# metagentools/VStrains

Measured on AMD Instinct MI355X. Metric: PE read pairs/sec through PE-link inference (GFA index + packed reads in HBM -> node_mat/short_mat), higher is better.
Workload: dtype u32

## Files before the change

include/vstrains_hip.h:

```cpp
#ifndef VSTRAINS_HIP_H
#define VSTRAINS_HIP_H

#include <stddef.h>
#include <stdint.h>

#ifdef __cplusplus
extern "C" {
#endif

#define VS_ABI_VERSION 10

enum {
    VS_OK = 0,
    VS_E_ARG = -1,
    VS_E_HIP = -2,
    VS_E_OOM = -3,
    VS_E_NODE_BASE = -4,
    VS_E_STATE = -5,
    VS_E_RANGE = -6,
    VS_E_UTF8 = -7,
    VS_E_KEY = -8,
    VS_E_FPE = -9,
    VS_E_RECURSION = -10
};
// ... 71 lines not shown
                   const uint32_t *cum, uint32_t n_strains, uint64_t seed, uint64_t first_pair,
                   uint64_t n_pairs, uint32_t read_len, uint32_t sub_thresh, uint32_t n_thresh,
                   vs_reads **out);

int vs_pe_count(vs_ctx *ctx, const vs_reads *reads, uint32_t *d_node_mat, uint32_t *d_short_mat,
                uint64_t *d_stats);

int vs_pe_count_tracked(vs_ctx *ctx, const vs_reads *reads, uint32_t *d_node_mat, uint32_t *d_short_mat,
                        uint64_t *d_stats, uint8_t *d_tile_map);
int vs_counts_zero_tracked(vs_ctx *ctx, uint32_t *d_node_mat, uint32_t *d_short_mat, uint32_t n, uint8_t *d_tile_map);

int vs_counts_fold(vs_ctx *ctx, uint32_t *d_counts, int64_t *d_wide, uint64_t n);

int vs_counts_occupied(vs_ctx *ctx, const void *d_cells, uint32_t cell_bytes, uint64_t n_stretches, uint8_t *d_occ);

int vs_comm_unique_id(vs_ctx *ctx, uint8_t id[128]);
int vs_comm_init_rank(vs_ctx *ctx, int n_ranks, const uint8_t id[128], int rank, void **comm);
int vs_comm_destroy(vs_ctx *ctx, void *comm);
int vs_pe_allreduce(vs_ctx *ctx, void *comm, void *d_node_mat, void *d_short_mat, uint64_t *d_stats,
                    uint32_t n, int wide);

int vs_pe_map_ends(vs_ctx *ctx, const vs_reads *reads, uint32_t cap, uint32_t *lists,
                   uint32_t *counts);

int vs_pe_last_timing(vs_ctx *ctx, double ms[5]);
const char *vs_pe_last_kernel(const vs_ctx *ctx);
enum {
    VS_RAN_LOCUS_LDS_SORT = 1,
    VS_RAN_LOCUS_GLOBAL_SORT = 2,
    VS_RAN_PE_MID = 8,
    VS_RAN_ROW_OWNERS = 16
};
uint32_t vs_pe_last_launched(const vs_ctx *ctx);

typedef struct vs_links vs_links;
int vs_links_from_counts(vs_ctx *ctx, const uint32_t *d_node_mat, const uint32_t *d_short_mat,
                         uint32_t n, vs_links **out);
int vs_links_from_counts_tracked(vs_ctx *ctx, const uint32_t *d_node_mat, const uint32_t *d_short_mat, uint32_t n,
                                 const uint8_t *d_tile_map, uint32_t sparse_min_nodes, vs_links **out);
int vs_links_from_wide(vs_ctx *ctx, const int64_t *d_node_mat, const int64_t *d_short_mat,
                       uint32_t n, vs_links **out);
int vs_links_from_host(vs_ctx *ctx, const int64_t *node_mat, const int64_t *short_mat, uint32_t n,
                       vs_links **out);
int vs_links_reserve(vs_ctx *ctx, uint32_t n);
void vs_links_free(vs_ctx *ctx, vs_links *links);
int vs_links_size(const vs_links *links, uint32_t *n);
int vs_links_to_host(vs_ctx *ctx, const vs_links *links, int64_t *out );
int vs_links_block_sums(vs_ctx *ctx, const vs_links *links, const uint64_t *list_off,
                        const uint32_t *list_idx, uint32_t n_lists, const uint32_t *qa,
                        const uint32_t *qb, uint64_t n_queries, int64_t *out);
int vs_links_group_matrix(vs_ctx *ctx, const vs_links *links, const uint64_t *list_off,
                          const uint32_t *list_idx, uint32_t n_groups, int64_t *out);

int vs_graph_refresh(vs_ctx *ctx, uint32_t n_vertices, uint32_t n_edge_slots,
                     const uint64_t *row_ptr, const uint32_t *n_out, const uint32_t *nbr,
                     const uint32_t *eidx, const double *dp, const uint8_t *vertex_black,
                     const uint8_t *edge_black, double *flow, uint8_t *nontrivial,
                     uint8_t *fork_kind, int32_t *chain_next, int32_t *chain_top,
                     int32_t *chain_rank, uint32_t *zero_sum_edge);

typedef struct vs_stage vs_stage;
enum {
    VS_STAGE_GRAPH = 1,
    VS_STAGE_CONTIGS = 2,
    VS_STAGE_LINKS = 4,
    VS_STAGE_STRAINS = 8,
// ... 38 lines not shown
```

vstrains_amd/_native.py:

```python
from __future__ import annotations

import ctypes as C
import os

_HERE = os.path.dirname(os.path.abspath(__file__))
LIB_PATH = os.path.join(_HERE, "libvstrains_hip.so")

VS_OK = 0
VS_E_ARG, VS_E_HIP, VS_E_OOM, VS_E_NODE_BASE, VS_E_STATE, VS_E_RANGE, VS_E_UTF8, VS_E_KEY, VS_E_FPE = -1, -2, -3, -4, -5, -6, -7, -8, -9

SYMBOLS = {
    "vs_abi_version": (C.c_int, []),
    "vs_device_count": (C.c_int, []),
    "vs_ctx_create": (C.c_int, [C.c_int, C.POINTER(C.c_void_p)]),
    "vs_ctx_destroy": (None, [C.c_void_p]),
    "vs_last_error": (C.c_char_p, [C.c_void_p]),
    "vs_ctx_set_stream": (C.c_int, [C.c_void_p, C.c_void_p]),
    "vs_ctx_sync": (C.c_int, [C.c_void_p]),
    "vs_index_build": (C.c_int, [C.c_void_p, C.c_void_p, C.c_void_p, C.c_uint32, C.c_uint32,
                                 C.POINTER(C.c_uint32), C.POINTER(C.c_uint8)]),
    "vs_index_info": (C.c_int, [C.c_void_p, C.POINTER(C.c_uint64)]),
    "vs_index_export": (C.c_int, [C.c_void_p, C.c_void_p, C.c_void_p, C.c_void_p, C.c_void_p, C.c_void_p, C.POINTER(C.c_uint64)]),
    "vs_node_order_host": (C.c_int, [C.c_void_p, C.c_void_p, C.c_uint32, C.c_uint32, C.c_void_p]),
    "vs_reads_pack": (C.c_int, [C.c_void_p, C.c_void_p, C.c_void_p, C.c_uint64, C.POINTER(C.c_void_p)]),
# ... 13 lines not shown
    "vs_fastq_block": (C.c_int, [C.c_void_p, C.c_void_p, C.c_uint64, C.c_uint64, C.POINTER(C.c_void_p)]),
    "vs_fastq_stream_open": (C.c_int, [C.c_void_p, C.c_char_p, C.c_char_p, C.POINTER(C.c_void_p)]),
    "vs_fastq_stream_next": (C.c_int, [C.c_void_p, C.c_void_p, C.c_uint64, C.POINTER(C.c_void_p), C.POINTER(C.c_uint64)]),
    "vs_fastq_stream_info": (C.c_int, [C.c_void_p, C.POINTER(C.c_uint64)]),
    "vs_fastq_stream_close": (None, [C.c_void_p]),
    "vs_fastq_scan_text": (C.c_int, [C.c_void_p, C.c_void_p, C.c_uint64, C.c_uint32, C.c_void_p, C.c_uint64, C.POINTER(C.c_uint64)]),
    "vs_bgzf_walk": (C.c_int, [C.c_void_p, C.c_uint64, C.c_void_p, C.c_uint64, C.POINTER(C.c_uint64)]),
    "vs_inflate_host": (C.c_int, [C.c_void_p, C.c_uint32, C.c_void_p, C.c_uint32, C.c_uint32, C.POINTER(C.c_uint32)]),
    "vs_inflate_bgzf": (C.c_int, [C.c_void_p, C.c_void_p, C.c_uint64, C.c_void_p, C.c_uint64, C.c_uint32, C.c_void_p, C.c_uint64,
                                  C.POINTER(C.c_uint64)]),
    "vs_fastq_stream_inflate_info": (C.c_int, [C.c_void_p, C.POINTER(C.c_uint64)]),
    "vs_bgzf_walk_file": (C.c_int, [C.c_char_p, C.c_void_p, C.c_uint64, C.POINTER(C.c_uint64)]),
    "vs_bgzf_count_lines": (C.c_int, [C.c_void_p, C.c_char_p, C.c_void_p, C.c_uint64, C.c_void_p, C.POINTER(C.c_uint64)]),
    "vs_inflate_count_host": (C.c_int, [C.c_void_p, C.c_uint32, C.c_uint32, C.c_uint32, C.POINTER(C.c_uint32)]),
    "vs_bgzf_shard_plan": (C.c_int, [C.c_void_p, C.c_uint64, C.c_int, C.c_uint64, C.c_uint64, C.POINTER(C.c_uint64)]),
    "vs_fastq_stream_open_range": (C.c_int, [C.c_void_p, C.c_char_p, C.c_char_p, C.POINTER(C.c_uint64), C.c_uint64, C.POINTER(C.c_void_p)]),
    "vs_write_matrix_text": (C.c_int, [C.c_void_p, C.c_char_p, C.c_void_p, C.c_void_p, C.c_uint32, C.c_void_p]),
    "vs_synth_pairs": (C.c_int, [C.c_void_p, C.c_void_p, C.c_void_p, C.c_void_p, C.c_uint32, C.c_uint64,
                                 C.c_uint64, C.c_uint64, C.c_uint32, C.c_uint32, C.c_uint32,
                                 C.POINTER(C.c_void_p)]),
    "vs_pe_count": (C.c_int, [C.c_void_p, C.c_void_p, C.c_void_p, C.c_void_p, C.c_void_p]),
    "vs_pe_count_tracked": (C.c_int, [C.c_void_p, C.c_void_p, C.c_void_p, C.c_void_p, C.c_void_p, C.c_void_p]),
    "vs_counts_zero_tracked": (C.c_int, [C.c_void_p, C.c_void_p, C.c_void_p, C.c_uint32, C.c_void_p]),
    "vs_counts_fold": (C.c_int, [C.c_void_p, C.c_void_p, C.c_void_p, C.c_uint64]),
    "vs_counts_occupied": (C.c_int, [C.c_void_p, C.c_void_p, C.c_uint32, C.c_uint64, C.c_void_p]),
    "vs_comm_unique_id": (C.c_int, [C.c_void_p, C.c_void_p]),
    "vs_comm_init_rank": (C.c_int, [C.c_void_p, C.c_int, C.c_void_p, C.c_int, C.POINTER(C.c_void_p)]),
    "vs_comm_destroy": (C.c_int, [C.c_void_p, C.c_void_p]),
    "vs_pe_allreduce": (C.c_int, [C.c_void_p, C.c_void_p, C.c_void_p, C.c_void_p, C.c_void_p, C.c_uint32, C.c_int]),
    "vs_pe_map_ends": (C.c_int, [C.c_void_p, C.c_void_p, C.c_uint32, C.c_void_p, C.c_void_p]),
    "vs_pe_last_kernel": (C.c_char_p, [C.c_void_p]),
    "vs_pe_last_launched": (C.c_uint32, [C.c_void_p]),
    "vs_pe_last_timing": (C.c_int, [C.c_void_p, C.POINTER(C.c_double)]),
    "vs_links_from_counts": (C.c_int, [C.c_void_p, C.c_void_p, C.c_void_p, C.c_uint32, C.POINTER(C.c_void_p)]),
    "vs_links_from_counts_tracked": (C.c_int, [C.c_void_p, C.c_void_p, C.c_void_p, C.c_uint32, C.c_void_p, C.c_uint32, C.POINTER(C.c_void_p)]),
    "vs_links_from_wide": (C.c_int, [C.c_void_p, C.c_void_p, C.c_void_p, C.c_uint32, C.POINTER(C.c_void_p)]),
    "vs_links_from_host": (C.c_int, [C.c_void_p, C.c_void_p, C.c_void_p, C.c_uint32, C.POINTER(C.c_void_p)]),
    "vs_links_reserve": (C.c_int, [C.c_void_p, C.c_uint32]),
    "vs_links_free": (None, [C.c_void_p, C.c_void_p]),
    "vs_links_size": (C.c_int, [C.c_void_p, C.POINTER(C.c_uint32)]),
    "vs_links_to_host": (C.c_int, [C.c_void_p, C.c_void_p, C.c_void_p]),
    "vs_links_block_sums": (C.c_int, [C.c_void_p, C.c_void_p, C.c_void_p, C.c_void_p, C.c_uint32, C.c_void_p,
                                      C.c_void_p, C.c_uint64, C.c_void_p]),
    "vs_links_group_matrix": (C.c_int, [C.c_void_p, C.c_void_p, C.c_void_p, C.c_void_p, C.c_uint32, C.c_void_p]),
    "vs_graph_refresh": (C.c_int, [C.c_void_p, C.c_uint32, C.c_uint32] + [C.c_void_p] * 13 + [C.POINTER(C.c_uint32)]),
    "vs_stage_create": (C.c_int, [C.c_void_p, C.c_void_p, C.POINTER(C.c_void_p)]),
    "vs_dev_alloc": (C.c_int, [C.c_void_p, C.c_size_t, C.POINTER(C.c_void_p)]),
    "vs_dev_free": (C.c_int, [C.c_void_p, C.c_void_p]),
    "vs_dev_zero": (C.c_int, [C.c_void_p, C.c_void_p, C.c_size_t]),
    "vs_dev_to_host": (C.c_int, [C.c_void_p, C.c_void_p, C.c_void_p, C.c_size_t]),
}

_lib = None


class NativeError(RuntimeError):
    def __init__(self, code: int, msg: str):
        super().__init__("libvstrains_hip: %s (code %d)" % (msg, code))
        self.code = code


def lib():
    global _lib
    if _lib is None:
        if not os.path.exists(LIB_PATH):
            raise ImportError(
# ... 20 lines not shown
```

vstrains_amd/csrc/vs_internal.h:

```cpp
#pragma once

#include <hip/hip_runtime.h>
#include <stdint.h>
#include <string>
#include <vector>

#include "../../include/vstrains_hip.h"
#include "vs_buf.h"
#include "vs_pe_plan.h"

#define VS_WAVE 64
#define VS_PAD_WORDS 16


struct VsNodeMeta {
    uint32_t woff;
    uint32_t len;
};

struct VsSlot {
    uint64_t key;
    uint32_t a;
    uint32_t b;
};
// ... 58 lines not shown

void vs_tuning_load(VsTuning &t, bool experiment);

struct vs_ctx {
    int device = 0;
    bool experiment = false;
    VsTuning tune;
    hipStream_t stream = nullptr;
    std::string err;
    FqStage fq_stage[2];
    unsigned fq_next = 0;
    bool has_index = false;
    VsIndexDev idx{};
    VsDevBuf d_meta, d_fwd, d_table, d_post;
    uint64_t n_seed_pos = 0, n_slots = 0, n_distinct = 0, index_bytes = 0;
    uint32_t max_node_len = 0;
    VsDevBuf d_slow_list;
    VsDevBuf d_slow_count;
    enum SlowCount : uint32_t {
        SC_MID = 0,
        SC_ACC_QUEUE = 1,
        SC_SLOW = 8,
        SC_STRIP_QUEUE = 9,
        SC_OWNERS = 15,
        SC_WORDS = 16
    };
    VsDevBuf links_spare;
    uint32_t links_spare_n = 0;
    VsDevBuf d_slow_list2;
    VsDevBuf d_dense;
    uint32_t dense_nodes = 0xFFFFFFFFu;
    VsDevBuf d_locus_keys, d_perm, d_locus_hist, d_scan_tmp;
    double last_sort_ms = 0;
    VsDevBuf d_lists, d_list_counts;
    VsDevBuf d_rows, d_row_entries, d_mult, d_ltab;
    VsDevBuf scratch[32];
    struct CachedBuf { VsDevBuf buf; bool used; };
    std::vector<CachedBuf> cache;
    hipEvent_t ev[5] = {nullptr, nullptr, nullptr, nullptr, nullptr};
    double last_ms[3] = {0, 0, 0};
    const char *last_kernel = "";
    uint32_t last_launched = 0;
    int n_cu = 256;
};

struct vs_reads {
    uint64_t n_ends = 0, n_words = 0, max_len = 0, n_invalid = 0, bytes = 0;
    void *d_woff = nullptr, *d_meta = nullptr, *d_words = nullptr, *d_mask = nullptr, *d_inv4 = nullptr;
    bool cached = false;
    VsDevBuf own[5];
    unsigned n_own = 0;
    hipError_t own_alloc(void *&view, size_t bytes) {
        const hipError_t e = own[n_own].reserve(bytes);
        view = own[n_own].ptr();
        if (e == hipSuccess) n_own++;
        return e;
    }
    VsReadsDev dev() const {
        VsReadsDev r;
        r.n_ends = n_ends;
        r.woff = (const uint32_t *)d_woff;
        r.meta = (const uint32_t *)d_meta;
        r.words = (const uint32_t *)d_words;
        r.mask = (const uint32_t *)d_mask;
        r.inv4 = (const uint32_t *)d_inv4;
        return r;
// ... 57 lines not shown
__device__ __forceinline__ uint64_t vs_win(const uint32_t *w, uint32_t base) { return vs_win64_u32(w, base); }
__device__ __forceinline__ uint64_t vs_win(const uint32_t *w, uint64_t base) { return vs_win64(w, base); }

__device__ __forceinline__ uint32_t vs_fastdiv(uint32_t x, uint32_t magic) { return magic ? __umulhi(x, magic) : x; }

__device__ __forceinline__ uint64_t vs_lowmask(uint32_t bits) {
    return bits >= 64u ? ~0ull : ((1ull << bits) - 1ull);
}

__device__ __forceinline__ uint64_t vs_rc(uint64_t x, uint32_t w) {
    x = __builtin_bitreverse64(x);
    x = ((x >> 1) & 0x5555555555555555ull) | ((x & 0x5555555555555555ull) << 1);
    return (~x) >> (64u - 2u * w);
}

__device__ __forceinline__ uint64_t vs_mix64(uint64_t z);
template <typename B>
__device__ __forceinline__ uint64_t vs_seed_key(const uint32_t *words, B base, uint32_t w, uint32_t *strand) {
    if (w <= 31u) {
        const uint64_t f = vs_win(words, base) & vs_lowmask(2u * w);
        const uint64_t r = vs_rc(f, w);
        *strand = r < f ? 1u : 0u;
        return r < f ? r : f;
    }
    const uint32_t sh = 2u * (w - 32u);
    const uint64_t lo = vs_win(words, base), hi = vs_win(words, base + (B)32) & vs_lowmask(sh);
    const uint64_t rl = vs_rc(lo, 32u), rh = vs_rc(hi, w - 32u);
    const uint64_t rc_lo = (rl << sh) | rh, rc_hi = sh ? rl >> (64u - sh) : 0ull;
    const bool rev = rc_hi < hi || (rc_hi == hi && rc_lo < lo);
    *strand = rev ? 1u : 0u;
    const uint64_t a = rev ? rc_lo : lo, b = rev ? rc_hi : hi;
    return vs_mix64(a ^ vs_mix64(b + 0x632BE59BD9B4E019ull)) >> 2;
}
template <typename B>
__device__ __forceinline__ bool vs_seed_dirty(const uint32_t *mask, B base, uint32_t w) {
    if (w <= 32u) return (vs_win(mask, base) & vs_lowmask(2u * w)) != 0ull;
    return vs_win(mask, base) != 0ull || (vs_win(mask, base + (B)32) & vs_lowmask(2u * (w - 32u))) != 0ull;
}

__device__ __forceinline__ uint32_t vs_slot_of(uint64_t key, uint32_t bits) {
    return (uint32_t)((key * 0x9E3779B97F4A7C15ull) >> (64u - bits));
}

__device__ __forceinline__ uint64_t vs_mix64(uint64_t z) {
    z += 0x9E3779B97F4A7C15ull;
    z = (z ^ (z >> 30)) * 0xBF58476D1CE4E5B9ull;
    z = (z ^ (z >> 27)) * 0x94D049BB133111EBull;
    return z ^ (z >> 31);
}

template <typename T>
__device__ __forceinline__ uint32_t vs_upper_idx(const T *a, uint32_t n, T x) {
    uint32_t lo = 0, hi = n;
    while (hi - lo > 1) {
        uint32_t mid = (lo + hi) >> 1;
        if (a[mid] <= x) lo = mid; else hi = mid;
    }
    return lo;
}

#endif
```

vstrains_amd/csrc/vs_pe.hip:

```cpp
#include <stdio.h>
#include <stdlib.h>
#include <string.h>

#include "vs_internal.h"

#define TPB 256
#define LCAP 20u
__device__ __forceinline__ const uint32_t *vs_row_quad(const uint32_t *__restrict__ lists, const uint32_t *__restrict__ hi, uint64_t row, uint32_t q) {
    return q < LC / 4u ? lists + row * LC + 4u * q : hi + row * 4u;
}
#define EMPTY_NODE 0xFFFFFFFFu

struct PeParams {
    VsIndexDev idx;
    VsReadsDev rd;
    uint32_t *node_mat, *short_mat;
    unsigned long long *stats;
    uint32_t ept, pmax, words_cap, pool, pool_bits;
    uint64_t n_tiles;
    uint32_t *slow_list, *slow_count;
    uint32_t *dbg_lists, *dbg_counts;
    uint32_t dbg_cap;
    uint32_t accumulate;
    const uint32_t *perm;
// ... 1460 lines not shown
__device__ __forceinline__ uint32_t vs_locus_key(const VsIndexDev &idx, const VsReadsDev &rd, uint64_t p) {
    const uint32_t mf = rd.meta[2 * p], mr = rd.meta[2 * p + 1];
    const uint32_t N = idx.n_nodes, w = idx.w, s = idx.s, K = idx.K;
    if ((((mf | mr) >> 24) & VS_FLAG_N) || (mf & VS_LEN_MASK) < K || (mr & VS_LEN_MASK) < K) return N + 1u;
    const uint32_t rlen = mf & VS_LEN_MASK;
    const uint64_t base = (uint64_t)rd.woff[2 * p] * 16u;
    const bool inv = (mf >> 24) & VS_FLAG_INVALID;
    for (uint32_t j = vs_seed_phase(rlen, w, s); j + w <= rlen; j += s) {
        if (inv && vs_seed_dirty(rd.mask, base + j, w)) continue;
        uint32_t pa, pb, sr;
        const uint64_t key = vs_seed_key(rd.words, base + j, w, &sr);
        const uint32_t c = vs_probe(idx, key, sr, &pa, &pb);
        if (c) return c == 1u ? pa : (idx.postings[pa].x & 0x01FFFFFFu);
    }
    return N;
}

__device__ __forceinline__ uint32_t vs_locus_key_end(const VsIndexDev &idx, const VsReadsDev &rd, uint64_t e) {
    const uint32_t m = rd.meta[e];
    const uint32_t N = idx.n_nodes, w = idx.w, s = idx.s, rlen = m & VS_LEN_MASK;
    const uint64_t base = (uint64_t)rd.woff[e] * 16u;
    const bool inv = (m >> 24) & VS_FLAG_INVALID;
    for (uint32_t j = vs_seed_phase(rlen, w, s); j + w <= rlen; j += s) {
        if (inv && vs_seed_dirty(rd.mask, base + j, w)) continue;
        uint32_t pa, pb, sr;
        const uint64_t key = vs_seed_key(rd.words, base + j, w, &sr);
        const uint32_t c = vs_probe(idx, key, sr, &pa, &pb);
        if (c) return c == 1u ? pa : (idx.postings[pa].x & 0x01FFFFFFu);
    }
    return N;
}

#define LOCUS_TPB 1024
__global__ void __launch_bounds__(LOCUS_TPB)
k_locus_count(VsIndexDev idx, VsReadsDev rd, uint64_t n_pairs, uint32_t chunk, uint32_t n_wg, uint32_t *__restrict__ keys,
              uint32_t *__restrict__ cnt, uint32_t key_lo, uint32_t nk, uint32_t compute) {
    for (uint32_t i = threadIdx.x; i < nk; i += LOCUS_TPB) vs_lds[i] = 0;
    __syncthreads();
    const uint64_t lo = (uint64_t)blockIdx.x * chunk;
    const uint64_t hi = lo + chunk < n_pairs ? lo + chunk : n_pairs;
    for (uint64_t p = lo + threadIdx.x; p < hi; p += LOCUS_TPB) {
        uint32_t key;
        if (compute) {
            key = vs_locus_key(idx, rd, p);
            keys[p] = key;
        } else {
            key = keys[p];
        }
        if (key - key_lo < nk) atomicAdd(&vs_lds[key - key_lo], 1u);
    }
    __syncthreads();
    for (uint32_t i = threadIdx.x; i < nk; i += LOCUS_TPB) cnt[(uint64_t)(key_lo + i) * n_wg + blockIdx.x] = vs_lds[i];
}

__global__ void __launch_bounds__(LOCUS_TPB)
k_locus_scatter(uint32_t key_lo, uint32_t nk, uint64_t n_pairs, uint32_t chunk, uint32_t n_wg, const uint32_t *__restrict__ keys,
                const uint32_t *__restrict__ first, uint32_t *__restrict__ perm) {
    for (uint32_t i = threadIdx.x; i < nk; i += LOCUS_TPB) vs_lds[i] = first[(uint64_t)(key_lo + i) * n_wg + blockIdx.x];
    __syncthreads();
    const uint64_t lo = (uint64_t)blockIdx.x * chunk;
    const uint64_t hi = lo + chunk < n_pairs ? lo + chunk : n_pairs;
    for (uint64_t p = lo + threadIdx.x; p < hi; p += LOCUS_TPB) {
        const uint32_t key = keys[p];
        if (key - key_lo < nk) perm[atomicAdd(&vs_lds[key - key_lo], 1u)] = (uint32_t)p;
    }
}

__global__ void __launch_bounds__(TPB)
k_pe_locus(VsIndexDev idx, VsReadsDev rd, uint64_t n_pairs, uint32_t *__restrict__ keys, uint32_t *__restrict__ hist) {
    const uint64_t p = (uint64_t)blockIdx.x * TPB + threadIdx.x;
    if (p >= n_pairs) return;
    const uint32_t key = vs_locus_key(idx, rd, p);
    keys[p] = key;
    atomicAdd(&hist[key], 1u);
}

__global__ void __launch_bounds__(TPB)
k_pe_permute(uint64_t n_pairs, const uint32_t *__restrict__ keys, uint32_t *__restrict__ cursor, uint32_t *__restrict__ perm) {
    const uint64_t p = (uint64_t)blockIdx.x * TPB + threadIdx.x;
    if (p >= n_pairs) return;
    perm[atomicAdd(&cursor[keys[p]], 1u)] = (uint32_t)p;
}
// ... 371 lines not shown
            const uint32_t off = (uint32_t)(((uintptr_t)m >> 2) & 15u);
            VS_HIP(ctx, hipMemsetAsync(queue, 0, sizeof(uint32_t), st));
            if (mode)
                hipLaunchKernelGGL(k_rows_sum<1>, dim3(grid), dim3(RS_TPB), RSUM_LDS_BYTES, st, sl, sh, sc, (const uint32_t *)mult, N, row_ptr, entries, R, n_strips, fill, m,
                                   off, d_tile_map, T, queue);
            else
                hipLaunchKernelGGL(k_rows_sum<0>, dim3(grid), dim3(RS_TPB), RSUM_LDS_BYTES, st, sl, sh, sc, (const uint32_t *)mult, N, row_ptr, entries, R, n_strips, fill, m,
                                   off, d_tile_map, T, queue);
        }
    }
    VS_HIP(ctx, hipGetLastError());
    return VS_OK;
}

struct TilesFn {
    uint32_t mode, sw, sp, ad;
    const void *fn;
    const char *name;
};
#define TILES(M, SW, SP) {M, SW, SP, 0u, (const void *)k_pe_tiles<M, SW, SP>, "k_pe_tiles<" #M ", " #SW ", " #SP ">"}
#define TILES_AD(M, SW, SP) {M, SW, SP, 1u, (const void *)k_pe_tiles<M, SW, SP, true>, "k_pe_tiles<" #M ", " #SW ", " #SP ", true>"}, TILES(M, SW, SP)
static const TilesFn TILES_TABLE[] = {TILES_AD(1, 10u, 4u), TILES_AD(1, 8u, 3u), TILES_AD(1, 7u, 2u), TILES_AD(1, 7u, 3u), TILES(1, 0u, 0u),
                                      TILES_AD(2, 16u, 2u), TILES(2, 0u, 0u),    TILES(0, 0u, 0u)};

static int pe_launch(vs_ctx *ctx, const vs_reads *reads, uint32_t *d_node_mat, uint32_t *d_short_mat, uint64_t *d_stats,
                     uint32_t *d_dbg_lists, uint32_t *d_dbg_counts, uint32_t dbg_cap, uint8_t *d_tile_map = nullptr) {
    if (!ctx->has_index) return vs_fail(ctx, VS_E_STATE, "vs_pe_count: build an index first (vs_index_build)");
    VS_HIP(ctx, hipSetDevice(ctx->device));
    hipStream_t st = ctx->stream;
    const VsIndexDev &idx = ctx->idx;
    const uint64_t n_pairs = reads->n_ends / 2;
    ctx->last_ms[0] = ctx->last_ms[1] = ctx->last_ms[2] = 0;
    ctx->last_launched = 0;
    if (ctx->experiment) vs_tuning_load(ctx->tune, true);
    PePlanIn in;
    in.n_nodes = idx.n_nodes; in.K = idx.K; in.w = idx.w; in.s = idx.s;
    in.n_seed_pos = ctx->n_seed_pos; in.n_distinct = ctx->n_distinct; in.max_node_len = ctx->max_node_len; in.n_cu = (uint32_t)ctx->n_cu;
    in.n_ends = reads->n_ends; in.max_len = (uint32_t)reads->max_len;
    in.has_mask = reads->d_mask != nullptr; in.has_inv4 = reads->d_inv4 != nullptr;
    in.count = d_node_mat != nullptr; in.tile_map = d_tile_map != nullptr;
    in.tune = ctx->tune;
    const PePlan pl = vs_pe_plan(in);
    if (pl.status != VS_OK) return vs_fail(ctx, pl.status, "%s", pl.msg);
    if (!pl.n_tiles) return VS_OK;
    const TilesFn *tf = nullptr;
    for (const TilesFn &t : TILES_TABLE)
        if (t.mode == pl.mode && t.sw == pl.sw && t.sp == pl.sp && t.ad == pl.ad) tf = &t;
    if (!tf) return vs_fail(ctx, VS_E_STATE, "vs_pe_count: the plan names k_pe_tiles<%u, %uu, %uu, %u>, which this build does not hold", pl.mode, pl.sw, pl.sp, pl.ad);

    VS_HIP(ctx, ctx->d_slow_list.reserve(sizeof(uint32_t) * n_pairs));
    VS_HIP(ctx, ctx->d_slow_count.reserve(sizeof(uint32_t) * vs_ctx::SC_WORDS));
    VS_HIP(ctx, ctx->d_slow_list2.reserve(sizeof(uint32_t) * n_pairs));
    if (ctx->dense_nodes != idx.n_nodes) ctx->d_dense.reset();
    bool dense_new = false;
    VS_HIP(ctx, ctx->d_dense.reserve(pl.dense_bytes, pl.dense_bytes, &dense_new));
    if (dense_new) {
        ctx->dense_nodes = idx.n_nodes;
        uint64_t N = idx.n_nodes ? idx.n_nodes : 1;
        VS_HIP(ctx, hipMemsetAsync(ctx->d_dense.ptr(), 0xFF, pl.dense_bytes, st));
        hipLaunchKernelGGL(k_dense_zero_cnt, dim3((unsigned)((N * pl.slow_grid + TPB - 1) / TPB)), dim3(TPB), 0, st,
                           ctx->d_dense.as<uint32_t>(), N, (uint64_t)pl.slow_grid);
    }
    VS_HIP(ctx, hipMemsetAsync(ctx->d_slow_count.ptr(), 0, sizeof(uint32_t) * vs_ctx::SC_WORDS, st));
    if (pl.use_sort) {
        VS_HIP(ctx, ctx->d_locus_keys.reserve(sizeof(uint32_t) * n_pairs));
        VS_HIP(ctx, ctx->d_perm.reserve(sizeof(uint32_t) * n_pairs));
// ... 46 lines not shown
        const uint64_t nk = pl.locus_keys;
        ctx->last_launched |= pl.lds_sort ? VS_RAN_LOCUS_LDS_SORT : VS_RAN_LOCUS_GLOBAL_SORT;
        if (pl.lds_sort) {
            const uint32_t n_wg = LOCUS_WGS, chunk = pl.locus_chunk, per_pass = pl.locus_per_pass;
            const size_t lds_keys = sizeof(uint32_t) * per_pass;
            if (lds_keys > 64u * 1024u) {
                VS_HIP(ctx, hipFuncSetAttribute((const void *)k_locus_count, hipFuncAttributeMaxDynamicSharedMemorySize, (int)lds_keys));
                VS_HIP(ctx, hipFuncSetAttribute((const void *)k_locus_scatter, hipFuncAttributeMaxDynamicSharedMemorySize, (int)lds_keys));
            }
            for (uint32_t key_lo = 0; key_lo < nk; key_lo += per_pass) {
                const uint32_t n_here = (uint32_t)(nk - key_lo < per_pass ? nk - key_lo : per_pass);
                hipLaunchKernelGGL(k_locus_count, dim3(n_wg), dim3(LOCUS_TPB), lds_keys, st, idx, reads->dev(), n_pairs, chunk, n_wg,
                                   ctx->d_locus_keys.as<uint32_t>(), ctx->d_locus_hist.as<uint32_t>(), key_lo, n_here, key_lo == 0u ? 1u : 0u);
            }
            int rc = vs_scan_u32(ctx, ctx->d_locus_hist.as<const uint32_t>(), ctx->d_locus_hist.as<uint32_t>(), nk * n_wg,
                                 ctx->d_scan_tmp.as<uint64_t>(), nullptr);
            if (rc) return rc;
            for (uint32_t key_lo = 0; key_lo < nk; key_lo += per_pass) {
                const uint32_t n_here = (uint32_t)(nk - key_lo < per_pass ? nk - key_lo : per_pass);
                hipLaunchKernelGGL(k_locus_scatter, dim3(n_wg), dim3(LOCUS_TPB), lds_keys, st, key_lo, n_here, n_pairs, chunk, n_wg,
                                   ctx->d_locus_keys.as<const uint32_t>(), ctx->d_locus_hist.as<const uint32_t>(), ctx->d_perm.as<uint32_t>());
            }
        } else {
            VS_HIP(ctx, hipMemsetAsync(ctx->d_locus_hist.ptr(), 0, sizeof(uint32_t) * nk, st));
            const unsigned pg = (unsigned)((n_pairs + TPB - 1) / TPB);
            hipLaunchKernelGGL(k_pe_locus, dim3(pg), dim3(TPB), 0, st, idx, reads->dev(), n_pairs, ctx->d_locus_keys.as<uint32_t>(),
                               ctx->d_locus_hist.as<uint32_t>());
            int rc = vs_scan_u32(ctx, ctx->d_locus_hist.as<const uint32_t>(), ctx->d_locus_hist.as<uint32_t>(), nk,
                                 ctx->d_scan_tmp.as<uint64_t>(), nullptr);
            if (rc) return rc;
            hipLaunchKernelGGL(k_pe_permute, dim3(pg), dim3(TPB), 0, st, n_pairs, ctx->d_locus_keys.as<const uint32_t>(),
                               ctx->d_locus_hist.as<uint32_t>(), ctx->d_perm.as<uint32_t>());
        }
    }
    VS_HIP(ctx, hipEventRecord(ctx->ev[0], st));
    if (!d_node_mat) VS_HIP(ctx, hipEventRecord(ctx->ev[4], st));
    ctx->last_kernel = tf->name;
    {
        void *kargs[] = {(void *)&P};
        VS_HIP(ctx, hipLaunchKernel(tf->fn, dim3((unsigned)pl.grid), dim3(TTPB), kargs, lds, st));
    }
    if (d_node_mat) {
        const uint64_t used_ends = 2ull * n_pairs;
        if (pl.list_ends > used_ends)
            VS_HIP(ctx, hipMemsetAsync(ctx->d_list_counts.as<uint32_t>() + used_ends, 0, sizeof(uint32_t) * (pl.list_ends - used_ends), st));
        const uint64_t slots_pairs = pl.list_ends / 2;
        VS_HIP(ctx, hipEventRecord(ctx->ev[4], st));
        if (pl.use_rows) {
            const int rc = pe_count_by_rows(ctx, pl, d_node_mat, d_short_mat, d_tile_map, P.tile_T);
            if (rc) return rc;
            ctx->last_launched |= VS_RAN_ROW_OWNERS;
        } else {
            uint32_t *acc_queue = ctx->d_slow_count.as<uint32_t>() + vs_ctx::SC_ACC_QUEUE;
            if (pl.mark_tiles)
                hipLaunchKernelGGL(k_mark_tiles, dim3((unsigned)((slots_pairs + 255u) / 256u)), dim3(256), 0, st, ctx->d_lists.as<const uint32_t>(),
                                   ctx->d_list_counts.as<const uint32_t>(), slots_pairs, d_tile_map, P.tile_T, pl.ept);
            VS_HIP(ctx, hipFuncSetAttribute((const void *)k_pe_accumulate, hipFuncAttributeMaxDynamicSharedMemorySize, (int)ACC_LDS_BYTES));
            hipLaunchKernelGGL(k_pe_accumulate, dim3(pl.acc_grid), dim3(ACC_TPB), ACC_LDS_BYTES, st, ctx->d_lists.as<const uint32_t>(),
                               ctx->d_list_counts.as<const uint32_t>(), slots_pairs, pl.acc_per_wg, idx.n_nodes, pl.use_table, pl.acc_fill, d_node_mat,
                               d_short_mat, acc_queue, pl.ept);
        }
    }
    VS_HIP(ctx, hipEventRecord(ctx->ev[1], st));
    const bool no_mid = ctx->tune.no_mid;
    ctx->last_launched |= no_mid ? 0u : VS_RAN_PE_MID;
    if (!no_mid) {
// ... 6 lines not shown
                           ctx->d_slow_list.as<const uint32_t>(), ctx->d_slow_count.as<const uint32_t>());
    }
    VS_HIP(ctx, hipEventRecord(ctx->ev[2], st));
    VS_HIP(ctx, hipGetLastError());
    return VS_OK;
}

extern "C" int vs_pe_count(vs_ctx *ctx, const vs_reads *reads, uint32_t *d_node_mat, uint32_t *d_short_mat, uint64_t *d_stats) {
    if (!ctx || !reads || !d_node_mat || !d_short_mat || !d_stats) return VS_E_ARG;
    return pe_launch(ctx, reads, d_node_mat, d_short_mat, d_stats, nullptr, nullptr, 0);
}

extern "C" int vs_pe_count_tracked(vs_ctx *ctx, const vs_reads *reads, uint32_t *d_node_mat, uint32_t *d_short_mat, uint64_t *d_stats,
                                   uint8_t *d_tile_map) {
    if (!ctx || !reads || !d_node_mat || !d_short_mat || !d_stats || !d_tile_map) return VS_E_ARG;
    return pe_launch(ctx, reads, d_node_mat, d_short_mat, d_stats, nullptr, nullptr, 0, d_tile_map);
}

extern "C" int vs_counts_zero_tracked(vs_ctx *ctx, uint32_t *d_node_mat, uint32_t *d_short_mat, uint32_t n, uint8_t *d_tile_map) {
    if (!ctx || (n && (!d_node_mat || !d_short_mat || !d_tile_map))) return vs_fail(ctx, VS_E_ARG, "vs_counts_zero_tracked: bad argument");
    if (!n) return VS_OK;
    VS_HIP(ctx, hipSetDevice(ctx->device));
    const uint32_t T = (n + 63u) >> 6;
    const uint64_t tiles = 2ull * T * T;
    if (tiles > 0x7FFFFFFFull) return vs_fail(ctx, VS_E_RANGE, "vs_counts_zero_tracked: %u nodes make more tiles than one launch takes", n);
    hipLaunchKernelGGL(k_zero_tiles, dim3((unsigned)((tiles + 63u) / 64u)), dim3(64), 0, ctx->stream, d_node_mat, d_short_mat, n, T, d_tile_map, tiles);
    VS_HIP(ctx, hipGetLastError());
    return VS_OK;
}

extern "C" const char *vs_pe_last_kernel(const vs_ctx *ctx) { return ctx ? ctx->last_kernel : ""; }
extern "C" uint32_t vs_pe_last_launched(const vs_ctx *ctx) { return ctx ? ctx->last_launched : 0u; }

extern "C" int vs_pe_last_timing(vs_ctx *ctx, double ms[5]) {
    if (!ctx || !ms) return VS_E_ARG;
    VS_HIP(ctx, hipSetDevice(ctx->device));
    VS_HIP(ctx, hipEventSynchronize(ctx->ev[2]));
    float a = 0, b = 0, c = 0, d = 0;
    VS_HIP(ctx, hipEventElapsedTime(&a, ctx->ev[0], ctx->ev[1]));
    VS_HIP(ctx, hipEventElapsedTime(&d, ctx->ev[4], ctx->ev[1]));
    if (d > a) d = 0;
    a -= d;
    VS_HIP(ctx, hipEventElapsedTime(&b, ctx->ev[1], ctx->ev[2]));
    VS_HIP(ctx, hipEventElapsedTime(&c, ctx->ev[3], ctx->ev[0]));
    ctx->last_sort_ms = c;
    uint32_t n_slow = 0;
    VS_HIP(ctx, hipMemcpy(&n_slow, ctx->d_slow_count.ptr(), sizeof n_slow, hipMemcpyDeviceToHost));
    ms[0] = a; ms[1] = b; ms[2] = (double)n_slow; ms[3] = c; ms[4] = d;
    ctx->last_ms[0] = a; ctx->last_ms[1] = b; ctx->last_ms[2] = n_slow;
    return VS_OK;
}

extern "C" int vs_pe_map_ends(vs_ctx *ctx, const vs_reads *reads, uint32_t cap, uint32_t *lists, uint32_t *counts) {
    if (!ctx || !reads || !lists || !counts || !cap) return VS_E_ARG;
    VS_HIP(ctx, hipSetDevice(ctx->device));
    uint64_t n = reads->n_ends;
    if (!n) return VS_OK;
    VsDevBuf lists_buf, counts_buf;
    VS_HIP(ctx, lists_buf.reserve(sizeof(uint32_t) * n * cap));
    VS_HIP(ctx, counts_buf.reserve(sizeof(uint32_t) * n));
    uint32_t *d_lists = lists_buf.as<uint32_t>(), *d_counts = counts_buf.as<uint32_t>();
    VS_HIP(ctx, hipMemsetAsync(d_counts, 0, sizeof(uint32_t) * n, ctx->stream));
    VS_HIP(ctx, hipMemsetAsync(d_lists, 0xFF, sizeof(uint32_t) * n * cap, ctx->stream));
    const int rc = pe_launch(ctx, reads, nullptr, nullptr, nullptr, d_lists, d_counts, cap);
    if (rc != VS_OK) return rc;
    VS_HIP(ctx, hipMemcpyAsync(lists, d_lists, sizeof(uint32_t) * n * cap, hipMemcpyDeviceToHost, ctx->stream));
// ... 5 lines not shown
```

vstrains_amd/pe.py:

```python
from __future__ import annotations

import ctypes as C
import os
from typing import List, Optional, Sequence, Tuple

import numpy as np

from . import _native as nat
from .dist import U32_LIMIT, ExchangeState


def _universal_newlines(raw: bytes) -> bytes:
    if b"\r" in raw:
        raw = raw.replace(b"\r\n", b"\n").replace(b"\r", b"\n")
    return raw


def read_gfa_segments(path: str) -> Tuple[List[str], List[str]]:
    with open(path, "rb") as fh:
        raw = _universal_newlines(fh.read())
    ids: List[str] = []
    seqs: List[str] = []
    pieces = raw.split(b"\n")
    last_has_nl = raw.endswith(b"\n")
# ... 585 lines not shown
    def synth_pairs(self, genomes: Sequence[str], cum: np.ndarray, seed: int, first_pair: int, n_pairs: int,
                    read_len: int, sub_thresh: int = 0, n_thresh: int = 0) -> ReadBlock:
        gd, go = encode_seqs(genomes)
        cum = np.ascontiguousarray(cum, dtype=np.uint32)
        h = C.c_void_p()
        nat.check(self._h, nat.lib().vs_synth_pairs(self._h, gd.ctypes.data, go.ctypes.data, cum.ctypes.data,
                                                    len(genomes), seed, first_pair, n_pairs, read_len,
                                                    sub_thresh, n_thresh, C.byref(h)))
        return ReadBlock(self, h)

    def pe_count(self, reads: ReadBlock, node_mat_ptr: int, short_mat_ptr: int, stats_ptr: int, tile_map_ptr: Optional[int] = None):
        if tile_map_ptr is not None:
            nat.check(self._h, nat.lib().vs_pe_count_tracked(self._h, reads._h, C.c_void_p(node_mat_ptr), C.c_void_p(short_mat_ptr),
                                                             C.c_void_p(stats_ptr), C.c_void_p(tile_map_ptr)))
            return
        nat.check(self._h, nat.lib().vs_pe_count(self._h, reads._h, C.c_void_p(node_mat_ptr),
                                                 C.c_void_p(short_mat_ptr), C.c_void_p(stats_ptr)))

    def last_timing(self):
        a = (C.c_double * 5)()
        nat.check(self._h, nat.lib().vs_pe_last_timing(self._h, a))
        return dict(main_ms=a[0], slow_ms=a[1], slow_pairs=int(a[2]), sort_ms=a[3], accumulate_ms=a[4])

    @property
    def last_kernel(self) -> str:
        return (nat.lib().vs_pe_last_kernel(self._h) or b"").decode()

    RAN_LOCUS_LDS_SORT, RAN_LOCUS_GLOBAL_SORT, RAN_PE_MID, RAN_ROW_OWNERS = 1, 2, 8, 16

    @property
    def last_launched(self) -> int:
        return int(nat.lib().vs_pe_last_launched(self._h))

    def map_ends(self, reads: ReadBlock, cap: int = 64) -> List[List[int]]:
        n = reads.info["ends"]
        lists = np.zeros((max(n, 1), cap), dtype=np.uint32)
        counts = np.zeros(max(n, 1), dtype=np.uint32)
        nat.check(self._h, nat.lib().vs_pe_map_ends(self._h, reads._h, cap, lists.ctypes.data, counts.ctypes.data))
        out = []
        for e in range(n):
            c = int(counts[e])
            if c > cap:
                raise ValueError("end %d has %d nodes, cap %d" % (e, c, cap))
            ids = lists[e, :c] if self.node_order is None else self.node_order[lists[e, :c]]
            out.append(sorted(int(x) for x in ids))
        return out


class PeCounter:

    TRACK_TILES_MIN_BYTES = 2 << 30

    def __init__(self, ctx: Context, device: Optional[str] = None, track_tiles: Optional[bool] = None):
        import torch

        self.torch = torch
        self.ctx = ctx
        self.device = torch.device(device or ("cuda:%d" % ctx.device))
        n = ctx.n_nodes
        self.n = n
        self.mats = torch.zeros((2, max(n, 1), max(n, 1)), dtype=torch.int32, device=self.device)
        if track_tiles is None:
            track_tiles = self.device.type == "cuda" and (self.mats.numel() * 4 >= self.TRACK_TILES_MIN_BYTES or os.environ.get("VS_TRACK_TILES") == "1")
        tiles = (max(n, 1) + 63) // 64
        self.tile_map = torch.zeros(2 * tiles * tiles, dtype=torch.uint8, device=self.device) if track_tiles else None
        self.stats = torch.zeros(3, dtype=torch.int64, device=self.device)
# ... 159 lines not shown
```

Before: 1.349 billion.

## Batch locus-key hash probes across four pairs per thread for memory-level parallelism

Measured after the change: 1.332 billion. 1.3% lower.

```diff
diff --git a/include/vstrains_hip.h b/include/vstrains_hip.h
--- a/include/vstrains_hip.h
+++ b/include/vstrains_hip.h
@@ -127,6 +127,7 @@
     VS_RAN_ROW_OWNERS = 16
 };
 uint32_t vs_pe_last_launched(const vs_ctx *ctx);
+int vs_pe_last_locus(vs_ctx *ctx, uint32_t *keys_out, uint32_t *perm_out, uint64_t n);
 
 typedef struct vs_links vs_links;
 int vs_links_from_counts(vs_ctx *ctx, const uint32_t *d_node_mat, const uint32_t *d_short_mat,
diff --git a/vstrains_amd/_native.py b/vstrains_amd/_native.py
--- a/vstrains_amd/_native.py
+++ b/vstrains_amd/_native.py
@@ -69,6 +69,7 @@
     "vs_pe_last_kernel": (C.c_char_p, [C.c_void_p]),
     "vs_pe_last_launched": (C.c_uint32, [C.c_void_p]),
     "vs_pe_last_timing": (C.c_int, [C.c_void_p, C.POINTER(C.c_double)]),
+    "vs_pe_last_locus": (C.c_int, [C.c_void_p, C.c_void_p, C.c_void_p, C.c_uint64]),
     "vs_links_from_counts": (C.c_int, [C.c_void_p, C.c_void_p, C.c_void_p, C.c_uint32, C.POINTER(C.c_void_p)]),
     "vs_links_from_counts_tracked": (C.c_int, [C.c_void_p, C.c_void_p, C.c_void_p, C.c_uint32, C.c_void_p, C.c_uint32, C.POINTER(C.c_void_p)]),
     "vs_links_from_wide": (C.c_int, [C.c_void_p, C.c_void_p, C.c_void_p, C.c_uint32, C.POINTER(C.c_void_p)]),
diff --git a/vstrains_amd/csrc/vs_internal.h b/vstrains_amd/csrc/vs_internal.h
--- a/vstrains_amd/csrc/vs_internal.h
+++ b/vstrains_amd/csrc/vs_internal.h
@@ -114,6 +114,7 @@
     uint32_t dense_nodes = 0xFFFFFFFFu;
     VsDevBuf d_locus_keys, d_perm, d_locus_hist, d_scan_tmp;
     double last_sort_ms = 0;
+    uint64_t last_locus_n = 0;
     VsDevBuf d_lists, d_list_counts;
     VsDevBuf d_rows, d_row_entries, d_mult, d_ltab;
     VsDevBuf scratch[32];
@@ -237,6 +238,18 @@
     const uint64_t a = rev ? rc_lo : lo, b = rev ? rc_hi : hi;
     return vs_mix64(a ^ vs_mix64(b + 0x632BE59BD9B4E019ull)) >> 2;
 }
+__device__ __forceinline__ uint64_t vs_seed_key_win(uint64_t win0, uint64_t win1, uint32_t w) {
+    if (w <= 31u) {
+        const uint64_t f = win0 & vs_lowmask(2u * w), r = vs_rc(f, w);
+        return r < f ? r : f;
+    }
+    const uint32_t sh = 2u * (w - 32u);
+    const uint64_t lo = win0, hi = win1 & vs_lowmask(sh);
+    const uint64_t rl = vs_rc(lo, 32u), rh = vs_rc(hi, w - 32u);
+    const uint64_t rc_lo = (rl << sh) | rh, rc_hi = sh ? rl >> (64u - sh) : 0ull;
+    const bool rev = rc_hi < hi || (rc_hi == hi && rc_lo < lo);
+    return vs_mix64((rev ? rc_lo : lo) ^ vs_mix64((rev ? rc_hi : hi) + 0x632BE59BD9B4E019ull)) >> 2;
+}
 template <typename B>
 __device__ __forceinline__ bool vs_seed_dirty(const uint32_t *mask, B base, uint32_t w) {
     if (w <= 32u) return (vs_win(mask, base) & vs_lowmask(2u * w)) != 0ull;
diff --git a/vstrains_amd/csrc/vs_pe.hip b/vstrains_amd/csrc/vs_pe.hip
--- a/vstrains_amd/csrc/vs_pe.hip
+++ b/vstrains_amd/csrc/vs_pe.hip
@@ -1516,22 +1516,130 @@
 }
 
 #define LOCUS_TPB 1024
+#define LOCUS_B 4u
+__device__ __forceinline__ void vs_loaded(uint32_t &x) { asm volatile("" : "+v"(x)); }
+__device__ __forceinline__ void vs_loaded(uint64_t &x) { asm volatile("" : "+v"(x)); }
+template <uint32_t B, bool LONG>
+__device__ __forceinline__ uint32_t vs_locus_keys_wide(const VsIndexDev &idx, const VsReadsDev &rd, const uint32_t (&p)[B], uint32_t (&key)[B]) {
+    const uint32_t N = idx.n_nodes, w = idx.w, s = idx.s, K = idx.K;
+    __builtin_assume(LONG == (w > 31u));
+    const uint32_t tmask = (1u << idx.table_bits) - 1u;
+    const uint4 *tab = (const uint4 *)idx.table;
+    constexpr uint32_t ALL = (1u << B) - 1u;
+    uint2 m[B];
+    uint32_t wo[B];
+#pragma unroll
+    for (uint32_t i = 0; i < B; i++) {
+        m[i] = *(const uint2 *)(rd.meta + 2ull * p[i]);
+        wo[i] = rd.woff[2ull * p[i]];
+    }
+    uint32_t j[B], d[B], rlen[B], done = 0u, masked = 0u, multi = 0u;
+#pragma unroll
+    for (uint32_t i = 0; i < B; i++) {
+        const uint32_t mf = m[i].x, mr = m[i].y;
+        rlen[i] = mf & VS_LEN_MASK;
+        d[i] = 0u;
+        j[i] = 0u;
+        key[i] = N;
+        if ((((mf | mr) >> 24) & VS_FLAG_N) || rlen[i] < K || (mr & VS_LEN_MASK) < K) {
+            key[i] = N + 1u;
+            done |= 1u << i;
+        } else if ((mf >> 24) & VS_FLAG_INVALID) {
+            done |= 1u << i;
+            masked |= 1u << i;
+        } else if (vs_seed_phase(rlen[i], w, s) + w > rlen[i]) {
+            done |= 1u << i;
+        } else {
+            j[i] = vs_seed_phase(rlen[i], w, s);
+        }
+    }
+    while (done != ALL) {
+        uint64_t win0[B], win1[B];
+#pragma unroll
+        for (uint32_t i = 0; i < B; i++) {
+            const uint32_t *q = rd.words + wo[i] + (j[i] >> 4);
+            win0[i] = vs_win64_u32(q, j[i] & 15u);
+            win1[i] = LONG ? vs_win64_u32(q + 2, j[i] & 15u) : 0ull;
+        }
+#pragma unroll
+        for (uint32_t i = 0; i < B; i++) {
+            vs_loaded(win0[i]);
+            if (LONG) vs_loaded(win1[i]);
+        }
+        uint64_t sk[B];
+        uint4 raw[B];
+#pragma unroll
+        for (uint32_t i = 0; i < B; i++) {
+            sk[i] = vs_seed_key_win(win0[i], win1[i], w);
+            raw[i] = tab[(vs_slot_of(sk[i], idx.table_bits) + d[i]) & tmask];
+        }
+#pragma unroll
+        for (uint32_t i = 0; i < B; i++) { vs_loaded(raw[i].x); vs_loaded(raw[i].y); vs_loaded(raw[i].z); }
+#pragma unroll
+        for (uint32_t i = 0; i < B; i++) {
+            if ((done >> i) & 1u) continue;
+            const uint64_t k = (uint64_t)raw[i].x | ((uint64_t)raw[i].y << 32);
+            if (k == VS_EMPTY_KEY) {
+                if (j[i] + s + w > rlen[i]) {
+                    done |= 1u << i;
+                } else {
+                    j[i] += s;
+                    d[i] = 0u;
+                }
+            } else if ((k & ~VS_MULTI_BIT) == sk[i]) {
+                key[i] = raw[i].z;
+                if (k & VS_MULTI_BIT) multi |= 1u << i;
+                done |= 1u << i;
+            } else {
+                d[i]++;
+            }
+        }
+    }
+    uint32_t node[B];
+#pragma unroll
+    for (uint32_t i = 0; i < B; i++) node[i] = (((multi >> i) & 1u) ? idx.postings + key[i] : tab)->x;
+#pragma unroll
+    for (uint32_t i = 0; i < B; i++) vs_loaded(node[i]);
+#pragma unroll
+    for (uint32_t i = 0; i < B; i++)
+        if ((multi >> i) & 1u) key[i] = node[i] & 0x01FFFFFFu;
+    return masked;
+}
+
 __global__ void __launch_bounds__(LOCUS_TPB)
 k_locus_count(VsIndexDev idx, VsReadsDev rd, uint64_t n_pairs, uint32_t chunk, uint32_t n_wg, uint32_t *__restrict__ keys,
               uint32_t *__restrict__ cnt, uint32_t key_lo, uint32_t nk, uint32_t compute) {
+    constexpr uint32_t B = LOCUS_B;
     for (uint32_t i = threadIdx.x; i < nk; i += LOCUS_TPB) vs_lds[i] = 0;
     __syncthreads();
     const uint64_t lo = (uint64_t)blockIdx.x * chunk;
     const uint64_t hi = lo + chunk < n_pairs ? lo + chunk : n_pairs;
-    for (uint64_t p = lo + threadIdx.x; p < hi; p += LOCUS_TPB) {
-        uint32_t key;
+    for (uint64_t p0 = lo + threadIdx.x; p0 < hi; p0 += B * LOCUS_TPB) {
+        uint32_t p[B], key[B], masked = 0u;
+#pragma unroll
+        for (uint32_t i = 0; i < B; i++) {
+            const uint64_t q = p0 + i * LOCUS_TPB;
+            p[i] = (uint32_t)(q < hi ? q : p0);
+        }
         if (compute) {
-            key = vs_locus_key(idx, rd, p);
-            keys[p] = key;
+            masked = idx.w > 31u ? vs_locus_keys_wide<B, true>(idx, rd, p, key) : vs_locus_keys_wide<B, false>(idx, rd, p, key);
         } else {
-            key = keys[p];
-        }
-        if (key - key_lo < nk) atomicAdd(&vs_lds[key - key_lo], 1u);
+#pragma unroll
+            for (uint32_t i = 0; i < B; i++) key[i] = keys[p[i]];
+        }
+#pragma unroll
+        for (uint32_t i = 0; i < B; i++) {
+            if (p0 + i * LOCUS_TPB >= hi || ((masked >> i) & 1u)) continue;
+            if (compute) keys[p[i]] = key[i];
+            if (key[i] - key_lo < nk) atomicAdd(&vs_lds[key[i] - key_lo], 1u);
+        }
+        for (; masked; masked &= masked - 1u) {
+            const uint64_t q = p0 + (uint32_t)__builtin_ctz(masked) * LOCUS_TPB;
+            if (q >= hi) continue;
+            const uint32_t k1 = vs_locus_key(idx, rd, q);
+            keys[q] = k1;
+            if (k1 - key_lo < nk) atomicAdd(&vs_lds[k1 - key_lo], 1u);
+        }
     }
     __syncthreads();
     for (uint32_t i = threadIdx.x; i < nk; i += LOCUS_TPB) cnt[(uint64_t)(key_lo + i) * n_wg + blockIdx.x] = vs_lds[i];
@@ -1969,6 +2077,7 @@
     const uint64_t n_pairs = reads->n_ends / 2;
     ctx->last_ms[0] = ctx->last_ms[1] = ctx->last_ms[2] = 0;
     ctx->last_launched = 0;
+    ctx->last_locus_n = 0;
     if (ctx->experiment) vs_tuning_load(ctx->tune, true);
     PePlanIn in;
     in.n_nodes = idx.n_nodes; in.K = idx.K; in.w = idx.w; in.s = idx.s;
@@ -2081,6 +2190,7 @@
             hipLaunchKernelGGL(k_pe_permute, dim3(pg), dim3(TPB), 0, st, n_pairs, ctx->d_locus_keys.as<const uint32_t>(),
                                ctx->d_locus_hist.as<uint32_t>(), ctx->d_perm.as<uint32_t>());
         }
+        ctx->last_locus_n = n_pairs;
     }
     VS_HIP(ctx, hipEventRecord(ctx->ev[0], st));
     if (!d_node_mat) VS_HIP(ctx, hipEventRecord(ctx->ev[4], st));
@@ -2153,6 +2263,19 @@
 extern "C" const char *vs_pe_last_kernel(const vs_ctx *ctx) { return ctx ? ctx->last_kernel : ""; }
 extern "C" uint32_t vs_pe_last_launched(const vs_ctx *ctx) { return ctx ? ctx->last_launched : 0u; }
 
+extern "C" int vs_pe_last_locus(vs_ctx *ctx, uint32_t *keys_out, uint32_t *perm_out, uint64_t n) {
+    if (!ctx || !keys_out || !perm_out) return VS_E_ARG;
+    if (!ctx->last_locus_n) return vs_fail(ctx, VS_E_STATE, "vs_pe_last_locus: the last vs_pe_count did not sort its pairs");
+    if (n != ctx->last_locus_n)
+        return vs_fail(ctx, VS_E_ARG, "vs_pe_last_locus: %llu pairs asked for, the last vs_pe_count sorted %llu", (unsigned long long)n,
+                       (unsigned long long)ctx->last_locus_n);
+    VS_HIP(ctx, hipSetDevice(ctx->device));
+    VS_HIP(ctx, hipStreamSynchronize(ctx->stream));
+    VS_HIP(ctx, hipMemcpy(keys_out, ctx->d_locus_keys.ptr(), sizeof(uint32_t) * n, hipMemcpyDeviceToHost));
+    VS_HIP(ctx, hipMemcpy(perm_out, ctx->d_perm.ptr(), sizeof(uint32_t) * n, hipMemcpyDeviceToHost));
+    return VS_OK;
+}
+
 extern "C" int vs_pe_last_timing(vs_ctx *ctx, double ms[5]) {
     if (!ctx || !ms) return VS_E_ARG;
     VS_HIP(ctx, hipSetDevice(ctx->device));
diff --git a/vstrains_amd/pe.py b/vstrains_amd/pe.py
--- a/vstrains_amd/pe.py
+++ b/vstrains_amd/pe.py
@@ -641,6 +641,12 @@
     def last_launched(self) -> int:
         return int(nat.lib().vs_pe_last_launched(self._h))
 
+    def last_locus(self, n_pairs: int):
+        keys = np.zeros(max(n_pairs, 1), dtype=np.uint32)
+        perm = np.zeros(max(n_pairs, 1), dtype=np.uint32)
+        nat.check(self._h, nat.lib().vs_pe_last_locus(self._h, keys.ctypes.data, perm.ctypes.data, n_pairs))
+        return keys[:n_pairs], perm[:n_pairs]
+
     def map_ends(self, reads: ReadBlock, cap: int = 64) -> List[List[int]]:
         n = reads.info["ends"]
         lists = np.zeros((max(n, 1), cap), dtype=np.uint32)
```
